# iden3/snarkjs

Hardware: NVIDIA H100
Metric: groth16_proofs_per_sec (higher is better)
Workload: dtype u32x8 (256-bit modular integers, 32-bit limbs)

## Files before the change

### snarkjs_b200/csrc/ec.cuh

```cuda
#pragma once
#include "fp.cuh"

namespace sb {

template <class P> struct Fp2 {
    typedef Fp<P> B;
    static constexpr bool HAS_MUL2 = false;
    B a, b;
    SB_HD static Fp2 one() { Fp2 r; r.a = B::one(); r.b = B::zero(); return r; }
    SB_HD static Fp2 inv(const Fp2& x) {
        B t = B::inv_binary(B::add(B::sqr(x.a), B::sqr(x.b)));
        Fp2 r; r.a = B::mul(x.a, t); r.b = B::neg(B::mul(x.b, t)); return r;
    }
    SB_HD static Fp2 zero() { Fp2 r; r.a = B::zero(); r.b = B::zero(); return r; }
    SB_HD bool is_zero() const { return a.is_zero() & b.is_zero(); }
    SB_HD bool operator==(const Fp2& o) const { return (a == o.a) & (b == o.b); }
    SB_HD static Fp2 add(const Fp2& x, const Fp2& y) { Fp2 r; r.a = B::add(x.a, y.a); r.b = B::add(x.b, y.b); return r; }
    SB_HD static Fp2 sub(const Fp2& x, const Fp2& y) { Fp2 r; r.a = B::sub(x.a, y.a); r.b = B::sub(x.b, y.b); return r; }
    SB_HD static Fp2 dbl(const Fp2& x) { Fp2 r; r.a = B::dbl(x.a); r.b = B::dbl(x.b); return r; }
    SB_HD static Fp2 neg(const Fp2& x) { Fp2 r; r.a = B::neg(x.a); r.b = B::neg(x.b); return r; }
    SB_HD static Fp2 cneg(const Fp2& x, bool f) { Fp2 r; r.a = B::cneg(x.a, f); r.b = B::cneg(x.b, f); return r; }
    SB_HD_NOINLINE static Fp2 mul(const Fp2& x, const Fp2& y) { return mul_i(x, y); }
    SB_HD_NOINLINE static Fp2 sqr(const Fp2& x) { return sqr_i(x); }
    SB_HD static Fp2 mul_i(const Fp2& x, const Fp2& y) {
#if defined(__CUDA_ARCH__) && defined(SB_FP2_LAZY)
        return mul_lazy(x, y);
#endif
        if constexpr (B::HAS_MUL2) {
            Fp2 r; r.a = B::mul2(x.a, y.a, x.b, B::neg(y.b)); r.b = B::mul2(x.a, y.b, x.b, y.a); return r;
        } else {
            B A = B::mul(x.a, y.a), Bb = B::mul(x.b, y.b);
            B C = B::mul(B::add(x.a, x.b), B::add(y.a, y.b));
            Fp2 r; r.a = B::sub(A, Bb); r.b = B::sub(B::sub(C, A), Bb); return r;
        }
    }
    SB_HD static Fp2 mul_lazy(const Fp2& x, const Fp2& y) {
        constexpr int N = B::N;
        uint32_t v0[2 * N], v1[2 * N], v2[2 * N], sa[N], sb[N];
        B::mul_wide(x.a.v, y.a.v, v0);
        B::mul_wide(x.b.v, y.b.v, v1);
        B::add_noreduce(x.a, x.b, sa); B::add_noreduce(y.a, y.b, sb);
        B::mul_wide(sa, sb, v2);
        B::wide_sub(v2, v0); B::wide_sub(v2, v1);
        uint32_t bw = B::wide_sub(v0, v1);
        B::wide_add_p_high(v0, bw);
        Fp2 r; r.a = B::redc_wide(v0); r.b = B::redc_wide(v2); return r;
    }
    SB_HD static Fp2 sqr_i(const Fp2& x) {
        B AB = B::mul(x.a, x.b);
        Fp2 r; r.a = B::mul(B::add(x.a, x.b), B::sub(x.a, x.b)); r.b = B::dbl(AB); return r;
    }
};

template <class F> struct Affine {
    F x, y;
    SB_HD bool is_inf() const { return x.is_zero() & y.is_zero(); }
};

template <class F> struct XYZZ {
    F x, y, zz, zzz;
    SB_HD static XYZZ inf() { XYZZ r; r.x = F::zero(); r.y = F::zero(); r.zz = F::zero(); r.zzz = F::zero(); return r; }
    SB_HD bool is_inf() const { return zz.is_zero(); }

    SB_HD_NOINLINE static XYZZ dbl_affine(const F& px, const F& py, const F& one) {
        XYZZ r;
        if (py.is_zero()) return inf();
        F U = F::dbl(py), V = F::sqr(U), W = F::mul(U, V), S = F::mul(px, V);
        F M = F::sqr(px); M = F::add(F::dbl(M), M);
        r.x = F::sub(F::sqr(M), F::dbl(S));
        r.y = F::sub(F::mul(M, F::sub(S, r.x)), F::mul(W, py));
        r.zz = V; r.zzz = W;
        (void)one;
        return r;
    }
    SB_HD_NOINLINE static XYZZ dbl(const XYZZ& p) {
        if (p.is_inf() || p.y.is_zero()) return inf();
        XYZZ r;
        F U = F::dbl(p.y), V = F::sqr(U), W = F::mul(U, V), S = F::mul(p.x, V);
        F M = F::sqr(p.x); M = F::add(F::dbl(M), M);
        r.x = F::sub(F::sqr(M), F::dbl(S));
        r.y = F::sub(F::mul(M, F::sub(S, r.x)), F::mul(W, p.y));
        r.zz = F::mul(V, p.zz); r.zzz = F::mul(W, p.zzz);
        return r;
    }
    SB_HD void add_affine(const F& qx, const F& qy, const F& one) {
        if (is_inf()) { x = qx; y = qy; zz = one; zzz = one; return; }
        F U2 = F::mul_i(qx, zz), S2 = F::mul_i(qy, zzz);
        F Pp = F::sub(U2, x), R = F::sub(S2, y);
        if (Pp.is_zero()) {
            if (R.is_zero()) *this = dbl_affine(qx, qy, one);
            else *this = inf();
            return;
        }
        F PP = F::sqr_i(Pp), PPP = F::mul_i(Pp, PP), Q = F::mul_i(x, PP);
        F X3 = F::sub(F::sub(F::sqr_i(R), PPP), F::dbl(Q));
        F Y3;
        if constexpr (F::HAS_MUL2) Y3 = F::mul2_i(R, F::sub(Q, X3), F::neg(y), PPP);
        else Y3 = F::sub(F::mul_i(R, F::sub(Q, X3)), F::mul_i(y, PPP));
        x = X3; y = Y3; zz = F::mul_i(zz, PP); zzz = F::mul_i(zzz, PPP);
    }
    SB_HD void add(const XYZZ& q) {
        if (q.is_inf()) return;
        if (is_inf()) { *this = q; return; }
        F U1 = F::mul(x, q.zz), U2 = F::mul(q.x, zz);
        F S1 = F::mul(y, q.zzz), S2 = F::mul(q.y, zzz);
        F Pp = F::sub(U2, U1), R = F::sub(S2, S1);
        if (Pp.is_zero()) {
            if (R.is_zero()) *this = dbl(*this);
            else *this = inf();
            return;
        }
        F PP = F::sqr(Pp), PPP = F::mul(Pp, PP), Q = F::mul(U1, PP);
        F X3 = F::sub(F::sub(F::sqr(R), PPP), F::dbl(Q));
        F Y3 = F::sub(F::mul(R, F::sub(Q, X3)), F::mul(S1, PPP));
        x = X3; y = Y3;
        zz = F::mul(F::mul(zz, q.zz), PP); zzz = F::mul(F::mul(zzz, q.zzz), PPP);
    }
};

}
```

### snarkjs_b200/csrc/msm.cuh

```cuda
#pragma once
#include <cuda_runtime.h>
#include "ec.cuh"
#include "msm_geom.h"

namespace sb {

static constexpr int MSM_SEG = 32;
static constexpr int MSM_ACC_THREADS = 128;
static constexpr int MSM_RED_CHUNK = 16;
static constexpr uint32_t MSM_INVALID_KEY = 0xffffffffu;
static constexpr int MSM_COUNTS_SEG = 8;


__host__ inline MsmGeom msm_choose(uint64_t n, uint32_t scalar_bytes, int fr_bits, bool precomp) {
    int eff = (int)(8 * scalar_bytes) < fr_bits ? (int)(8 * scalar_bytes) : fr_bits;
    int best_c = 3; double best = 1e300;
    for (int c = 3; c <= 22; c++) {
        int weff = (eff + 1 + c - 1) / c, top = eff + 1 - (weff - 1) * c;
        if (weff > 1 && top < c - 5) continue;
        double buckets = (precomp ? 1.0 : (double)weff) * (double)(1u << (c - 1));
        double cost = (double)weff * (double)n * 10.0 + buckets * 60.0;
        if (cost < best) { best = cost; best_c = c; }
    }
    MsmGeom g; g.c = best_c; g.W = (int)((8 * scalar_bytes + 1 + best_c - 1) / best_c); g.B = 1u << (best_c - 1);
    return g;
}
__host__ inline MsmGeom msm_geometry_precomp(uint64_t n_set, uint32_t scalar_bytes, int fr_bits = 254) {
    int l2 = 0; while ((1ull << (l2 + 1)) <= n_set) l2++;
    int cmax = l2; if (cmax > 22) cmax = 22; if (cmax < 8) cmax = 8;
    int c = 8;
    for (int cc = cmax; cc >= 8; cc--) {
        int weff = (fr_bits + 1 + cc - 1) / cc, top = fr_bits + 1 - (weff - 1) * cc;
        if (weff > 1 && top < cc - 5) continue;
        c = cc; break;
    }
    MsmGeom g; g.c = c; g.W = (int)((8 * scalar_bytes + 1 + c - 1) / c); g.B = 1u << (c - 1);
    g.precomp = 1; g.stride = n_set; g.first = 0;
    return g;
}
__host__ inline MsmGeom msm_geometry(uint64_t n, uint32_t scalar_bytes, int fr_bits = 254) {
    return msm_choose(n, scalar_bytes, fr_bits, false);
}

template <class F> __device__ __forceinline__ void load_affine(const Affine<F>* __restrict__ bases, uint32_t idx, F& x, F& y) {
    constexpr int NV = sizeof(F) / 16;
    const uint4* p = reinterpret_cast<const uint4*>(bases + idx);
    uint4* dx = reinterpret_cast<uint4*>(&x);
    uint4* dy = reinterpret_cast<uint4*>(&y);
#pragma unroll
    for (int k = 0; k < NV; k++) dx[k] = __ldg(p + k);
#pragma unroll
    for (int k = 0; k < NV; k++) dy[k] = __ldg(p + NV + k);
}
template <class T> __device__ __forceinline__ void store_vec(T* dst, const T& v) {
    constexpr int NV = sizeof(T) / 16;
    const uint4* s = reinterpret_cast<const uint4*>(&v);
    uint4* d = reinterpret_cast<uint4*>(dst);
#pragma unroll
    for (int k = 0; k < NV; k++) d[k] = s[k];
}
template <class T> __device__ __forceinline__ T load_vec(const T* src) {
    constexpr int NV = sizeof(T) / 16;
    T v; const uint4* s = reinterpret_cast<const uint4*>(src);
    uint4* d = reinterpret_cast<uint4*>(&v);
#pragma unroll
    for (int k = 0; k < NV; k++) d[k] = s[k];
    return v;
}

template <class P> __device__ __forceinline__ Fp<P> PairInvF(const Fp<P>& a) { return Fp<P>::inv_binary(a); }
template <class P> __device__ __forceinline__ Fp2<P> PairInvF(const Fp2<P>& a) { return Fp2<P>::inv(a); }

template <class F, int MINB>
__global__ void __launch_bounds__(MSM_ACC_THREADS, MINB)
k_accumulate(const Affine<F>* __restrict__ bases, const uint32_t* __restrict__ keys, const uint32_t* __restrict__ vals,
             const uint64_t* __restrict__ counts, XYZZ<F>* __restrict__ buckets,
             XYZZ<F>* __restrict__ heads, uint32_t* __restrict__ head_keys) {
    const uint64_t M = counts[0];
    const uint32_t seg = (uint32_t)counts[MSM_COUNTS_SEG];
    uint64_t t = blockIdx.x * (uint64_t)blockDim.x + threadIdx.x;
    uint64_t lo = t * seg;
    if (lo >= M) return;
    uint64_t hi = lo + seg < M ? lo + seg : M;
    const F one = F::one();
    XYZZ<F> acc = XYZZ<F>::inf();
    uint32_t cur = keys[lo];
    bool first = true;
    for (uint64_t e = lo; e < hi; e++) {
        uint32_t k = keys[e], v = vals ? vals[e] : (uint32_t)e;
        if (k != cur) {
            if (first) { store_vec(heads + t, acc); head_keys[t] = cur; first = false; }
            else store_vec(buckets + cur, acc);
            acc = XYZZ<F>::inf(); cur = k;
        }
        F px, py;
        load_affine<F>(bases, v & 0x7fffffffu, px, py);
        if (!(px.is_zero() & py.is_zero())) {
            py = F::cneg(py, (v >> 31) != 0);
            acc.add_affine(px, py, one);
        }
    }
    if (first) { store_vec(heads + t, acc); head_keys[t] = cur; }
    else store_vec(buckets + cur, acc);
}

static constexpr int MSM_SHORT_RUN = 8;
template <class F>
__global__ void __launch_bounds__(MSM_ACC_THREADS)
k_fold_short(const XYZZ<F>* __restrict__ heads, const uint32_t* __restrict__ keys_in, uint32_t* __restrict__ keys_out,
             const uint64_t* __restrict__ counts, XYZZ<F>* __restrict__ buckets) {
    const uint64_t M = counts[1];
    uint64_t t = blockIdx.x * (uint64_t)blockDim.x + threadIdx.x;
    if (t >= M) return;
    const uint32_t k = keys_in[t];
    uint64_t start = t; int back = 0;
    while (start > 0 && back < MSM_SHORT_RUN && keys_in[start - 1] == k) { start--; back++; }
    bool is_short = back < MSM_SHORT_RUN;
    uint64_t len = 0;
    if (is_short) {
        len = 1;
        while (start + len < M && len <= (uint64_t)MSM_SHORT_RUN && keys_in[start + len] == k) len++;
        is_short = len <= (uint64_t)MSM_SHORT_RUN;
    }
    keys_out[t] = is_short ? MSM_INVALID_KEY : k;
    if (!is_short || start != t) return;
    XYZZ<F> acc = load_vec(buckets + k);
    for (uint64_t e = 0; e < len; e++) { XYZZ<F> p = load_vec(heads + t + e); acc.add(p); }
    store_vec(buckets + k, acc);
}

template <class F>
__global__ void __launch_bounds__(MSM_ACC_THREADS)
k_fold(const XYZZ<F>* __restrict__ in, const uint32_t* __restrict__ in_keys, const uint64_t* __restrict__ counts, int level,
       XYZZ<F>* __restrict__ buckets, XYZZ<F>* __restrict__ heads, uint32_t* __restrict__ head_keys) {
    const uint64_t M = counts[level];
    const bool last = M <= MSM_SEG;
    uint64_t t = blockIdx.x * (uint64_t)blockDim.x + threadIdx.x;
    uint64_t lo = t * MSM_SEG;
    if (lo >= M) return;
    uint64_t hi = lo + MSM_SEG < M ? lo + MSM_SEG : M;
    XYZZ<F> acc = XYZZ<F>::inf();
    uint32_t cur = in_keys[lo];
    bool first = !last;
    auto flush = [&]() {
        if (first) { store_vec(heads + t, acc); head_keys[t] = cur; first = false; }
        else if (cur != MSM_INVALID_KEY) { XYZZ<F> b = load_vec(buckets + cur); b.add(acc); store_vec(buckets + cur, b); }
    };
    for (uint64_t e = lo; e < hi; e++) {
        uint32_t k = in_keys[e];
        if (k != cur) { flush(); acc = XYZZ<F>::inf(); cur = k; }
        if (k != MSM_INVALID_KEY) { XYZZ<F> p = load_vec(in + e); acc.add(p); }
    }
    flush();
}

template <class F>
__global__ void __launch_bounds__(128)
k_reduce(const XYZZ<F>* __restrict__ buckets, MsmGeom g, XYZZ<F>* __restrict__ partials, uint32_t ctas_per_window) {
    extern __shared__ uint4 smem_raw[];
    XYZZ<F>* sm = reinterpret_cast<XYZZ<F>*>(smem_raw);
    const uint32_t w = blockIdx.x / ctas_per_window, cta = blockIdx.x % ctas_per_window;
    const uint32_t L = g.B < (uint32_t)MSM_RED_CHUNK ? g.B : MSM_RED_CHUNK;
    const uint32_t chunks = g.B / L;
    const uint32_t j = cta * blockDim.x + threadIdx.x;
    XYZZ<F> part = XYZZ<F>::inf();
    if (j < chunks) {
        const XYZZ<F>* bk = buckets + (uint64_t)w * g.B + (uint64_t)j * L;
        XYZZ<F> run = XYZZ<F>::inf(), sum = XYZZ<F>::inf();
        for (int b = (int)L - 1; b >= 0; b--) {
            XYZZ<F> p = load_vec(bk + b);
            run.add(p);
            sum.add(run);
        }
        uint32_t k = j * L;
        if (k) {
            int top = 31 - __clz(k);
            part = run;
            for (int bit = top - 1; bit >= 0; bit--) {
                part = XYZZ<F>::dbl(part);
                if ((k >> bit) & 1) part.add(run);
            }
        }
        part.add(sum);
    }
    store_vec(sm + threadIdx.x, part);
    __syncthreads();
    for (uint32_t s = blockDim.x >> 1; s > 0; s >>= 1) {
        if (threadIdx.x < s) {
            XYZZ<F> a = load_vec(sm + threadIdx.x), b = load_vec(sm + threadIdx.x + s);
            a.add(b);
            store_vec(sm + threadIdx.x, a);
        }
        __syncthreads();
    }
    if (threadIdx.x == 0) store_vec(partials + (uint64_t)w * ctas_per_window + cta, load_vec(sm));
}

template <class F>
__global__ void __launch_bounds__(32)
k_window_sum(const XYZZ<F>* __restrict__ partials, uint32_t per_window, XYZZ<F>* __restrict__ out) {
    extern __shared__ uint4 smem_raw[];
    XYZZ<F>* sm = reinterpret_cast<XYZZ<F>*>(smem_raw);
    XYZZ<F> acc = XYZZ<F>::inf();
    for (uint32_t i = threadIdx.x; i < per_window; i += 32) { XYZZ<F> p = load_vec(partials + (uint64_t)blockIdx.x * per_window + i); acc.add(p); }
    store_vec(sm + threadIdx.x, acc);
    __syncwarp();
    for (uint32_t s = 16; s > 0; s >>= 1) {
        if (threadIdx.x < s) { XYZZ<F> a = load_vec(sm + threadIdx.x), b = load_vec(sm + threadIdx.x + s); a.add(b); store_vec(sm + threadIdx.x, a); }
        __syncwarp();
    }
    if (threadIdx.x == 0) store_vec(out + blockIdx.x, load_vec(sm));
}

template <class F> __device__ __noinline__ void padd(XYZZ<F>& a, const XYZZ<F>& b) { a.add(b); }

struct AxisJob { const void* in; void* out; uint64_t total; uint32_t S; uint32_t log_inner; };

template <class F>
__global__ void __launch_bounds__(128)
k_axis_sum(AxisJob j0, AxisJob j1) {
    const AxisJob j = blockIdx.y ? j1 : j0;
    const uint64_t gid = blockIdx.x * (uint64_t)blockDim.x + threadIdx.x;
    if (gid >= j.total) return;
    const uint64_t o = gid >> j.log_inner, i = gid & ((1ull << j.log_inner) - 1);
    const XYZZ<F>* p = (const XYZZ<F>*)j.in + ((o * j.S) << j.log_inner) + i;
    XYZZ<F> acc = load_vec(p);
#pragma unroll 1
    for (uint32_t s = 1; s < j.S; s++) { XYZZ<F> v = load_vec(p + ((uint64_t)s << j.log_inner)); acc.add(v); }
    store_vec((XYZZ<F>*)j.out + gid, acc);
}

template <class F> __device__ __forceinline__ XYZZ<F> shfl_down_pt(const XYZZ<F>& v, int d) {
    constexpr int NW32 = sizeof(XYZZ<F>) / 4;
    union U { XYZZ<F> p; uint32_t w[NW32]; __device__ U() {} };
    U a, r; a.p = v;
#pragma unroll
    for (int k = 0; k < NW32; k++) r.w[k] = __shfl_down_sync(0xffffffffu, a.w[k], d);
    return r.p;
}
template <class F> __device__ __forceinline__ void warp_weighted_sum(XYZZ<F> v, XYZZ<F>& T, XYZZ<F>& W) {
    const int lane = threadIdx.x & 31;
#pragma unroll 1
    for (int d = 1; d < 32; d <<= 1) { XYZZ<F> o = shfl_down_pt<F>(v, d); if (lane + d < 32) v.add(o); }
    T = v;
    XYZZ<F> x = lane ? v : XYZZ<F>::inf();
#pragma unroll 1
    for (int d = 16; d >= 1; d >>= 1) { XYZZ<F> o = shfl_down_pt<F>(x, d); if (lane < d) x.add(o); }
    W = x;
}
template <class F> __device__ __forceinline__ XYZZ<F> warp_sum(XYZZ<F> x) {
    const int lane = threadIdx.x & 31;
#pragma unroll 1
    for (int d = 16; d >= 1; d >>= 1) { XYZZ<F> o = shfl_down_pt<F>(x, d); if (lane < d) x.add(o); }
    return x;
}

template <class F>
__global__ void __launch_bounds__(128)
k_ws_chunks(const XYZZ<F>* __restrict__ vecR, uint32_t lenR, const XYZZ<F>* __restrict__ vecC, uint32_t lenC, uint32_t NW, XYZZ<F>* __restrict__ tw) {
    const uint32_t nR = (lenR + 31) / 32, nC = (lenC + 31) / 32, per = nR + nC;
    const uint32_t wid = blockIdx.x * (blockDim.x >> 5) + (threadIdx.x >> 5), lane = threadIdx.x & 31;
    if (wid >= NW * per) return;
    const uint32_t w = wid / per, jj = wid % per;
    const bool isR = jj < nR;
    const uint32_t j = isR ? jj : jj - nR, len = isR ? lenR : lenC, idx = j * 32 + lane;
    const XYZZ<F>* vec = (isR ? vecR : vecC) + (uint64_t)w * len;
    XYZZ<F> v = XYZZ<F>::inf();
    if (idx < len) v = load_vec(vec + idx);
    XYZZ<F> T, W;
    warp_weighted_sum<F>(v, T, W);
    if (lane == 0) { store_vec(tw + 2 * (uint64_t)wid, T); store_vec(tw + 2 * (uint64_t)wid + 1, W); }
}

template <class F>
__global__ void __launch_bounds__(128)
k_ws_final(const XYZZ<F>* __restrict__ tw, uint32_t nR, uint32_t nC, XYZZ<F>* __restrict__ out) {
    const uint32_t warp = threadIdx.x >> 5, lane = threadIdx.x & 31, per = nR + nC;
    const XYZZ<F>* base = tw + 2 * (uint64_t)blockIdx.x * per;
    const bool r_side = warp < 2;
    const uint32_t cnt = r_side ? nR : nC, off = r_side ? 0 : nR;
    XYZZ<F> v = XYZZ<F>::inf();
    if (lane < cnt) v = load_vec(base + 2 * (uint64_t)(off + lane) + (warp & 1));
    XYZZ<F>* o = out + 5 * (uint64_t)blockIdx.x;
    if ((warp & 1) == 0) {
        XYZZ<F> tot, res;
        warp_weighted_sum<F>(v, tot, res);
        if (lane == 0) { store_vec(o + (r_side ? 0 : 2), res); if (!r_side) store_vec(o + 4, tot); }
    } else {
        XYZZ<F> res = warp_sum<F>(v);
        if (lane == 0) store_vec(o + (r_side ? 1 : 3), res);
    }
}

template <class F>
__global__ void __launch_bounds__(128)
k_axis_tree(AxisJob j0, AxisJob j1) {
    const AxisJob j = blockIdx.y ? j1 : j0;
    const uint64_t wid = blockIdx.x * (uint64_t)(blockDim.x >> 5) + (threadIdx.x >> 5);
    const uint32_t lane = threadIdx.x & 31;
    if (wid >= j.total) return;
    const uint64_t o = wid >> j.log_inner, i = wid & ((1ull << j.log_inner) - 1);
    const XYZZ<F>* p = (const XYZZ<F>*)j.in + ((o * j.S) << j.log_inner) + i;
    XYZZ<F> acc = XYZZ<F>::inf();
#pragma unroll 1
    for (uint32_t s = lane; s < j.S; s += 32) { XYZZ<F> v = load_vec(p + ((uint64_t)s << j.log_inner)); acc.add(v); }
    acc = warp_sum<F>(acc);
    if (lane == 0) store_vec((XYZZ<F>*)j.out + wid, acc);
}

static constexpr int WS_COL_BITS = 10;
struct WsPlan {
    bool ok = false;
    int m = 0, er = 0, ec = 0;
    int levels = 0; int br[8] = {0}, bc[8] = {0};
    uint32_t lenR = 0, lenC = 0, nR = 0, nC = 0;
    size_t rowA = 0, rowB = 0, colA = 0, colB = 0, tw = 0;
    size_t elems() const { return rowA + rowB + colA + colB + tw + 8; }
};
__host__ inline WsPlan ws_plan(const MsmGeom& g) {
    WsPlan p; const int cbits = g.c - 1; const size_t NW = g.windows();
    if (cbits > 2 * WS_COL_BITS || cbits < 0) return p;
    p.ok = true;
    if (cbits > WS_COL_BITS) { p.m = WS_COL_BITS; p.er = p.m; p.ec = cbits - p.m; p.lenR = 1u << p.ec; p.lenC = 1u << p.m; }
    else { p.lenR = 0; p.lenC = g.B; }
    int rr = p.er, rc = p.ec;
    for (int l = 0; l < 2 && (rr > 0 || rc > 0); l++) {
        p.levels++;
        p.br[l] = l == 0 ? (rr < 3 ? rr : 3) : rr; p.bc[l] = l == 0 ? (rc < 3 ? rc : 3) : rc; rr -= p.br[l]; rc -= p.bc[l];
        const size_t orow = p.br[l] ? (NW * g.B) >> (p.er - rr) : 0, ocol = p.bc[l] ? (NW * g.B) >> (p.ec - rc) : 0;
        if (l & 1) { p.rowB = orow; p.colB = ocol; } else { p.rowA = orow; p.colA = ocol; }
    }
    p.nR = (p.lenR + 31) / 32; p.nC = (p.lenC + 31) / 32;
    p.tw = 2 * NW * (p.nR + p.nC);
    return p;
}
__host__ inline size_t msm_reduce_scratch_elems(const MsmGeom& g) {
    const uint32_t NW = g.windows();
    const uint32_t L = g.B < (uint32_t)MSM_RED_CHUNK ? g.B : MSM_RED_CHUNK;
    const uint32_t ctas_per_window = (g.B / L + 127) / 128;
    const size_t legacy = (size_t)2 * NW * ctas_per_window;
    const WsPlan p = ws_plan(g);
    return (p.ok && p.elems() > legacy) ? p.elems() : legacy;
}

template <class F>
__global__ void __launch_bounds__(128) k_precompute(const Affine<F>* __restrict__ bases, uint64_t n, int c, int W, Affine<F>* __restrict__ table) {
    uint64_t i = blockIdx.x * (uint64_t)blockDim.x + threadIdx.x;
    if (i >= n) return;
    Affine<F> a = load_vec(bases + i);
    store_vec(table + i, a);
    if (a.is_inf()) {
        for (int w = 1; w < W; w++) store_vec(table + (uint64_t)w * n + i, a);
        return;
    }
    XYZZ<F> p; p.x = a.x; p.y = a.y; p.zz = F::one(); p.zzz = F::one();
    for (int w = 1; w < W; w++) {
        for (int j = 0; j < c; j++) p = XYZZ<F>::dbl(p);
        Affine<F> o;
        if (p.is_inf()) { o.x = F::zero(); o.y = F::zero(); }
        else { F t = PairInvF(F::mul(p.zz, p.zzz)); o.x = F::mul(p.x, F::mul(t, p.zzz)); o.y = F::mul(p.y, F::mul(t, p.zz)); p.x = o.x; p.y = o.y; p.zz = F::one(); p.zzz = F::one(); }
        store_vec(table + (uint64_t)w * n + i, o);
    }
}

__host__ __device__ inline uint64_t splitmix64(uint64_t x) {
    x += 0x9E3779B97F4A7C15ull; x = (x ^ (x >> 30)) * 0xBF58476D1CE4E5B9ull; x = (x ^ (x >> 27)) * 0x94D049BB133111EBull; return x ^ (x >> 31);
}
static constexpr uint64_t GEN_CHUNK = 4096;
template <class F>
__global__ void __launch_bounds__(128) k_gen_points(Affine<F> g, uint64_t seed, uint64_t n, Affine<F>* __restrict__ out) {
    uint64_t i = blockIdx.x * (uint64_t)blockDim.x + threadIdx.x;
    if (i >= n) return;
    const uint64_t c = i / GEN_CHUNK, j = i % GEN_CHUNK;
    const uint64_t k0 = (seed ^ 0x9E3779B97F4A7C15ull) + c * 0xD1B54A32D192ED03ull, kd = seed * 2654435761ull + 12345ull;
    uint64_t lo = j * kd, hi = __umul64hi(j, kd);
    lo += k0; hi += lo < k0 ? 1 : 0;
    const F one = F::one();
    XYZZ<F> r = XYZZ<F>::inf();
    for (int bit = 79; bit >= 0; bit--) {
        r = XYZZ<F>::dbl(r);
        const uint64_t wd = bit >= 64 ? hi : lo;
        if ((wd >> (bit & 63)) & 1) r.add_affine(g.x, g.y, one);
    }
    Affine<F> a;
    if (r.is_inf()) { a.x = F::zero(); a.y = F::zero(); }
    else { F t = PairInvF(F::mul(r.zz, r.zzz)); a.x = F::mul(r.x, F::mul(t, r.zzz)); a.y = F::mul(r.y, F::mul(t, r.zz)); }
    store_vec(out + i, a);
}

struct MsmScratch {
    void* p = nullptr; size_t cap = 0;
    void* get(size_t bytes) {
        if (bytes > cap) { if (p) cudaFree(p); p = nullptr; cap = 0; if (cudaMalloc(&p, bytes) != cudaSuccess) return nullptr; cap = bytes; }
        return p;
    }
    void release() { if (p) cudaFree(p); p = nullptr; cap = 0; }
};

extern int g_msm_force_reduce;

struct MsmLaunchStats {
    int launches = 0;
    cudaEvent_t* ev = nullptr; int nev = 0; int used = 0; int tag[128] = {0}; int cur_tag = 0;
};
enum { PROF_ACC_G1 = 1, PROF_ACC_G2 = 2, PROF_SORT = 3, PROF_FOLD = 4, PROF_REDUCE = 5, PROF_QAP = 6, PROF_NTT = 7, PROF_JOIN = 8 };
struct ProfScope {
    MsmLaunchStats* s; cudaStream_t st; int idx = -1;
    ProfScope(MsmLaunchStats* s_, int tag, cudaStream_t st_) : s(s_), st(st_) {
        if (s && s->ev && s->used + 2 <= s->nev && s->used / 2 < 128) { idx = s->used; s->used += 2; s->tag[idx / 2] = tag; cudaEventRecord(s->ev[idx], st); }
    }
    void end() { if (idx >= 0) { cudaEventRecord(s->ev[idx + 1], st); idx = -1; } }
    void end(cudaStream_t other) { st = other; end(); }
};

struct MsmSorted {
    const uint32_t* keys = nullptr; const uint32_t* vals = nullptr; const uint64_t* counts = nullptr;
    uint64_t n = 0, total = 0; MsmGeom g{};
    uint32_t seg_lo = MSM_SEG;
};

int msm_sort_entries(const uint8_t* d_scalars, uint32_t sbytes, uint64_t n, MsmGeom g, MsmScratch& scratch,
                     cudaStream_t stream, MsmSorted* out, MsmLaunchStats* stats);

template <class F>
int msm_buckets(const Affine<F>* d_bases, const MsmSorted& s, MsmScratch& scratch, cudaStream_t stream,
                XYZZ<F>* d_wsum, MsmLaunchStats* stats, cudaStream_t tail_stream = nullptr, cudaEvent_t ev_acc = nullptr) {
    const MsmGeom g = s.g;
    const uint32_t NW = g.windows();
    const uint64_t nbuckets = (uint64_t)NW * g.B;
    const uint64_t heads0 = (s.total + s.seg_lo - 1) / s.seg_lo;
    const uint64_t heads1 = (heads0 + MSM_SEG - 1) / MSM_SEG;
    const uint32_t L = g.B < (uint32_t)MSM_RED_CHUNK ? g.B : MSM_RED_CHUNK;
    const uint32_t chunks = g.B / L;
    const uint32_t red_threads = 128;
    const uint32_t ctas_per_window = (chunks + red_threads - 1) / red_threads;
    auto al = [](size_t x) { return (x + 255) & ~(size_t)255; };
    size_t o_buckets = 0;
    size_t o_headsA = o_buckets + al(nbuckets * sizeof(XYZZ<F>)), o_hkA = o_headsA + al(heads0 * sizeof(XYZZ<F>));
    size_t o_headsB = o_hkA + al(heads0 * 4), o_hkB = o_headsB + al(heads1 * sizeof(XYZZ<F>));
    size_t o_hkM = o_hkB + al(heads1 * 4);
    size_t o_part = o_hkM + al(heads0 * 4);
    size_t bytes = o_part + al(msm_reduce_scratch_elems(g) * sizeof(XYZZ<F>));
    uint8_t* base = (uint8_t*)scratch.get(bytes);
    if (!base) return (int)cudaErrorMemoryAllocation;
    XYZZ<F>* buckets = (XYZZ<F>*)(base + o_buckets);
    XYZZ<F>* headsA = (XYZZ<F>*)(base + o_headsA); uint32_t* hkA = (uint32_t*)(base + o_hkA);
    XYZZ<F>* headsB = (XYZZ<F>*)(base + o_headsB); uint32_t* hkB = (uint32_t*)(base + o_hkB);
    XYZZ<F>* partials = (XYZZ<F>*)(base + o_part);
    uint32_t* hkM = (uint32_t*)(base + o_hkM);
    int launches = 0;
    cudaMemsetAsync(buckets, 0, nbuckets * sizeof(XYZZ<F>), stream);
    if (heads0) {
        ProfScope prof(stats, stats ? stats->cur_tag : 0, stream);
        {
            const unsigned grid = (unsigned)((heads0 + MSM_ACC_THREADS - 1) / MSM_ACC_THREADS);
            constexpr int MINB = sizeof(F) > 32 ? 2 : 4;
            k_accumulate<F, MINB><<<grid, MSM_ACC_THREADS, 0, stream>>>(d_bases, s.keys, s.vals, s.counts, buckets, headsA, hkA);
            launches++;
        }
        prof.end();
        if (tail_stream && tail_stream != stream && ev_acc) {
            cudaEventRecord(ev_acc, stream); cudaStreamWaitEvent(tail_stream, ev_acc, 0); stream = tail_stream;
        }
        ProfScope pfold(stats, PROF_FOLD, stream);
        k_fold_short<F><<<(unsigned)((heads0 + MSM_ACC_THREADS - 1) / MSM_ACC_THREADS), MSM_ACC_THREADS, 0, stream>>>(
            headsA, hkA, hkM, s.counts, buckets); launches++;
        uint64_t m = heads0; int level = 1;
        XYZZ<F>* hin = headsA; uint32_t* kin = hkM; XYZZ<F>* hout = headsB; uint32_t* kout = hkB;
        while (true) {
            uint64_t threads = (m + MSM_SEG - 1) / MSM_SEG;
            k_fold<F><<<(unsigned)((threads + MSM_ACC_THREADS - 1) / MSM_ACC_THREADS), MSM_ACC_THREADS, 0, stream>>>(
                hin, kin, s.counts, level, buckets, hout, kout); launches++;
            if (m <= (uint64_t)MSM_SEG) break;
            m = threads; level++;
            XYZZ<F>* th = hin; hin = hout; hout = th; uint32_t* tk = kin; kin = kout; kout = tk;
            if (level >= 8) return (int)cudaErrorUnknown;
        }
        pfold.end();
    }
    if (!heads0 && tail_stream && tail_stream != stream && ev_acc) { cudaEventRecord(ev_acc, stream); cudaStreamWaitEvent(tail_stream, ev_acc, 0); stream = tail_stream; }
    ProfScope pred(stats, PROF_REDUCE, stream);
    const WsPlan wp = ws_plan(g);
    if (wp.ok && !g_msm_force_reduce) {
        XYZZ<F>* rowb[2] = {partials, partials + wp.rowA};
        XYZZ<F>* colb[2] = {partials + wp.rowA + wp.rowB, partials + wp.rowA + wp.rowB + wp.colA};
        XYZZ<F>* tw = partials + wp.rowA + wp.rowB + wp.colA + wp.colB;
        const XYZZ<F>* rin = buckets; const XYZZ<F>* cin = buckets;
        int rr = wp.er, rc = wp.ec;
        for (int l = 0; l < wp.levels; l++) {
            AxisJob jr{nullptr, nullptr, 0, 1, 0}, jc{nullptr, nullptr, 0, 1, 0};
            if (wp.br[l]) { rr -= wp.br[l]; jr = AxisJob{rin, rowb[l & 1], (uint64_t)nbuckets >> (wp.er - rr), 1u << wp.br[l], (uint32_t)rr}; rin = rowb[l & 1]; }
            if (wp.bc[l]) { rc -= wp.bc[l]; jc = AxisJob{cin, colb[l & 1], (uint64_t)nbuckets >> (wp.ec - rc), 1u << wp.bc[l], (uint32_t)wp.m}; cin = colb[l & 1]; }
            const uint64_t mx = jr.total > jc.total ? jr.total : jc.total;
            if (l == 0) k_axis_sum<F><<<dim3((unsigned)((mx + 127) / 128), 2), 128, 0, stream>>>(jr, jc);
            else k_axis_tree<F><<<dim3((unsigned)((mx + 3) / 4), 2), 128, 0, stream>>>(jr, jc);
            launches++;
        }
        const uint32_t per = wp.nR + wp.nC;
        k_ws_chunks<F><<<(NW * per + 3) / 4, 128, 0, stream>>>(wp.lenR ? rin : nullptr, wp.lenR, cin, wp.lenC, NW, tw); launches++;
        k_ws_final<F><<<NW, 128, 0, stream>>>(tw, wp.nR, wp.nC, d_wsum); launches++;
    } else {
        k_reduce<F><<<NW * ctas_per_window, red_threads, red_threads * sizeof(XYZZ<F>), stream>>>(buckets, g, partials, ctas_per_window); launches++;
        k_window_sum<F><<<NW, 32, 32 * sizeof(XYZZ<F>), stream>>>(partials, ctas_per_window, d_wsum); launches++;
    }
    pred.end();
    if (stats) stats->launches += launches;
    return (int)cudaGetLastError();
}

}
```

Measured before the change: 40.63.

## Inline XYZZ add, add minBlocks launch bounds, and simplify tail reductions

Rewrites the generic XYZZ point add to use the inlined field mul/sqr variants and the fused mul2 path. It precomputes ZZ/ZZZ and feeds the doubling case the normalized point. It adds minimum-blocks launch bounds to the fold, axis and weighted-sum kernels, switches load/store helpers to union-based vector copies to avoid address-taken locals, and restructures the warp weighted-sum into suffix-sum plus shared warp_sum calls. The goal is to cut call overhead and local-memory spills in the MSM tail kernels. The cost is higher register pressure from inlining, which the launch bounds may turn into spills, plus two extra field muls per add when the points are equal.

```diff
diff --git a/snarkjs_b200/csrc/ec.cuh b/snarkjs_b200/csrc/ec.cuh
--- a/snarkjs_b200/csrc/ec.cuh
+++ b/snarkjs_b200/csrc/ec.cuh
@@ -102,19 +102,20 @@
     SB_HD void add(const XYZZ& q) {
         if (q.is_inf()) return;
         if (is_inf()) { *this = q; return; }
-        F U1 = F::mul(x, q.zz), U2 = F::mul(q.x, zz);
-        F S1 = F::mul(y, q.zzz), S2 = F::mul(q.y, zzz);
-        F Pp = F::sub(U2, U1), R = F::sub(S2, S1);
+        F U1 = F::mul_i(x, q.zz), S1 = F::mul_i(y, q.zzz);
+        F Pp = F::sub(F::mul_i(q.x, zz), U1), R = F::sub(F::mul_i(q.y, zzz), S1);
+        F ZZ = F::mul_i(zz, q.zz), ZZZ = F::mul_i(zzz, q.zzz);
         if (Pp.is_zero()) {
-            if (R.is_zero()) *this = dbl(*this);
+            if (R.is_zero()) { XYZZ t; t.x = U1; t.y = S1; t.zz = ZZ; t.zzz = ZZZ; *this = dbl(t); }
             else *this = inf();
             return;
         }
-        F PP = F::sqr(Pp), PPP = F::mul(Pp, PP), Q = F::mul(U1, PP);
-        F X3 = F::sub(F::sub(F::sqr(R), PPP), F::dbl(Q));
-        F Y3 = F::sub(F::mul(R, F::sub(Q, X3)), F::mul(S1, PPP));
-        x = X3; y = Y3;
-        zz = F::mul(F::mul(zz, q.zz), PP); zzz = F::mul(F::mul(zzz, q.zzz), PPP);
+        F PP = F::sqr_i(Pp), PPP = F::mul_i(Pp, PP), Q = F::mul_i(U1, PP);
+        F X3 = F::sub(F::sub(F::sqr_i(R), PPP), F::dbl(Q));
+        F Y3;
+        if constexpr (F::HAS_MUL2) Y3 = F::mul2_i(R, F::sub(Q, X3), F::neg(S1), PPP);
+        else Y3 = F::sub(F::mul_i(R, F::sub(Q, X3)), F::mul_i(S1, PPP));
+        x = X3; y = Y3; zz = F::mul_i(ZZ, PP); zzz = F::mul_i(ZZZ, PPP);
     }
 };
 
diff --git a/snarkjs_b200/csrc/msm.cuh b/snarkjs_b200/csrc/msm.cuh
--- a/snarkjs_b200/csrc/msm.cuh
+++ b/snarkjs_b200/csrc/msm.cuh
@@ -10,6 +10,7 @@
 static constexpr int MSM_RED_CHUNK = 16;
 static constexpr uint32_t MSM_INVALID_KEY = 0xffffffffu;
 static constexpr int MSM_COUNTS_SEG = 8;
+template <class F> constexpr int MSM_TAIL_MINB = sizeof(F) == 32 ? 3 : 2;
 
 
 __host__ inline MsmGeom msm_choose(uint64_t n, uint32_t scalar_bytes, int fr_bits, bool precomp) {
@@ -42,30 +43,30 @@
     return msm_choose(n, scalar_bytes, fr_bits, false);
 }
 
+template <class T> union Vec16 { T v; uint4 u[sizeof(T) / 16]; __device__ Vec16() {} };
 template <class F> __device__ __forceinline__ void load_affine(const Affine<F>* __restrict__ bases, uint32_t idx, F& x, F& y) {
     constexpr int NV = sizeof(F) / 16;
     const uint4* p = reinterpret_cast<const uint4*>(bases + idx);
-    uint4* dx = reinterpret_cast<uint4*>(&x);
-    uint4* dy = reinterpret_cast<uint4*>(&y);
+    Vec16<F> dx, dy;
 #pragma unroll
-    for (int k = 0; k < NV; k++) dx[k] = __ldg(p + k);
+    for (int k = 0; k < NV; k++) dx.u[k] = __ldg(p + k);
 #pragma unroll
-    for (int k = 0; k < NV; k++) dy[k] = __ldg(p + NV + k);
+    for (int k = 0; k < NV; k++) dy.u[k] = __ldg(p + NV + k);
+    x = dx.v; y = dy.v;
 }
 template <class T> __device__ __forceinline__ void store_vec(T* dst, const T& v) {
     constexpr int NV = sizeof(T) / 16;
-    const uint4* s = reinterpret_cast<const uint4*>(&v);
+    Vec16<T> s; s.v = v;
     uint4* d = reinterpret_cast<uint4*>(dst);
 #pragma unroll
-    for (int k = 0; k < NV; k++) d[k] = s[k];
+    for (int k = 0; k < NV; k++) d[k] = s.u[k];
 }
 template <class T> __device__ __forceinline__ T load_vec(const T* src) {
     constexpr int NV = sizeof(T) / 16;
-    T v; const uint4* s = reinterpret_cast<const uint4*>(src);
-    uint4* d = reinterpret_cast<uint4*>(&v);
+    Vec16<T> d; const uint4* s = reinterpret_cast<const uint4*>(src);
 #pragma unroll
-    for (int k = 0; k < NV; k++) d[k] = s[k];
-    return v;
+    for (int k = 0; k < NV; k++) d.u[k] = s[k];
+    return d.v;
 }
 
 template <class P> __device__ __forceinline__ Fp<P> PairInvF(const Fp<P>& a) { return Fp<P>::inv_binary(a); }
@@ -106,7 +107,7 @@
 
 static constexpr int MSM_SHORT_RUN = 8;
 template <class F>
-__global__ void __launch_bounds__(MSM_ACC_THREADS)
+__global__ void __launch_bounds__(MSM_ACC_THREADS, MSM_TAIL_MINB<F>)
 k_fold_short(const XYZZ<F>* __restrict__ heads, const uint32_t* __restrict__ keys_in, uint32_t* __restrict__ keys_out,
              const uint64_t* __restrict__ counts, XYZZ<F>* __restrict__ buckets) {
     const uint64_t M = counts[1];
@@ -130,7 +131,7 @@
 }
 
 template <class F>
-__global__ void __launch_bounds__(MSM_ACC_THREADS)
+__global__ void __launch_bounds__(MSM_ACC_THREADS, MSM_TAIL_MINB<F>)
 k_fold(const XYZZ<F>* __restrict__ in, const uint32_t* __restrict__ in_keys, const uint64_t* __restrict__ counts, int level,
        XYZZ<F>* __restrict__ buckets, XYZZ<F>* __restrict__ heads, uint32_t* __restrict__ head_keys) {
     const uint64_t M = counts[level];
@@ -212,12 +213,10 @@
     if (threadIdx.x == 0) store_vec(out + blockIdx.x, load_vec(sm));
 }
 
-template <class F> __device__ __noinline__ void padd(XYZZ<F>& a, const XYZZ<F>& b) { a.add(b); }
-
 struct AxisJob { const void* in; void* out; uint64_t total; uint32_t S; uint32_t log_inner; };
 
 template <class F>
-__global__ void __launch_bounds__(128)
+__global__ void __launch_bounds__(MSM_ACC_THREADS, MSM_TAIL_MINB<F>)
 k_axis_sum(AxisJob j0, AxisJob j1) {
     const AxisJob j = blockIdx.y ? j1 : j0;
     const uint64_t gid = blockIdx.x * (uint64_t)blockDim.x + threadIdx.x;
@@ -238,15 +237,11 @@
     for (int k = 0; k < NW32; k++) r.w[k] = __shfl_down_sync(0xffffffffu, a.w[k], d);
     return r.p;
 }
-template <class F> __device__ __forceinline__ void warp_weighted_sum(XYZZ<F> v, XYZZ<F>& T, XYZZ<F>& W) {
+template <class F> __device__ __forceinline__ XYZZ<F> warp_suffix_sum(XYZZ<F> v) {
     const int lane = threadIdx.x & 31;
 #pragma unroll 1
     for (int d = 1; d < 32; d <<= 1) { XYZZ<F> o = shfl_down_pt<F>(v, d); if (lane + d < 32) v.add(o); }
-    T = v;
-    XYZZ<F> x = lane ? v : XYZZ<F>::inf();
-#pragma unroll 1
-    for (int d = 16; d >= 1; d >>= 1) { XYZZ<F> o = shfl_down_pt<F>(x, d); if (lane < d) x.add(o); }
-    W = x;
+    return v;
 }
 template <class F> __device__ __forceinline__ XYZZ<F> warp_sum(XYZZ<F> x) {
     const int lane = threadIdx.x & 31;
@@ -256,7 +251,7 @@
 }
 
 template <class F>
-__global__ void __launch_bounds__(128)
+__global__ void __launch_bounds__(MSM_ACC_THREADS, MSM_TAIL_MINB<F>)
 k_ws_chunks(const XYZZ<F>* __restrict__ vecR, uint32_t lenR, const XYZZ<F>* __restrict__ vecC, uint32_t lenC, uint32_t NW, XYZZ<F>* __restrict__ tw) {
     const uint32_t nR = (lenR + 31) / 32, nC = (lenC + 31) / 32, per = nR + nC;
     const uint32_t wid = blockIdx.x * (blockDim.x >> 5) + (threadIdx.x >> 5), lane = threadIdx.x & 31;
@@ -267,13 +262,14 @@
     const XYZZ<F>* vec = (isR ? vecR : vecC) + (uint64_t)w * len;
     XYZZ<F> v = XYZZ<F>::inf();
     if (idx < len) v = load_vec(vec + idx);
-    XYZZ<F> T, W;
-    warp_weighted_sum<F>(v, T, W);
-    if (lane == 0) { store_vec(tw + 2 * (uint64_t)wid, T); store_vec(tw + 2 * (uint64_t)wid + 1, W); }
-}
-
-template <class F>
-__global__ void __launch_bounds__(128)
+    v = warp_suffix_sum<F>(v);
+    if (lane == 0) store_vec(tw + 2 * (uint64_t)wid, v);
+    v = warp_sum<F>(lane ? v : XYZZ<F>::inf());
+    if (lane == 0) store_vec(tw + 2 * (uint64_t)wid + 1, v);
+}
+
+template <class F>
+__global__ void __launch_bounds__(MSM_ACC_THREADS, MSM_TAIL_MINB<F>)
 k_ws_final(const XYZZ<F>* __restrict__ tw, uint32_t nR, uint32_t nC, XYZZ<F>* __restrict__ out) {
     const uint32_t warp = threadIdx.x >> 5, lane = threadIdx.x & 31, per = nR + nC;
     const XYZZ<F>* base = tw + 2 * (uint64_t)blockIdx.x * per;
@@ -283,17 +279,16 @@
     if (lane < cnt) v = load_vec(base + 2 * (uint64_t)(off + lane) + (warp & 1));
     XYZZ<F>* o = out + 5 * (uint64_t)blockIdx.x;
     if ((warp & 1) == 0) {
-        XYZZ<F> tot, res;
-        warp_weighted_sum<F>(v, tot, res);
-        if (lane == 0) { store_vec(o + (r_side ? 0 : 2), res); if (!r_side) store_vec(o + 4, tot); }
-    } else {
-        XYZZ<F> res = warp_sum<F>(v);
-        if (lane == 0) store_vec(o + (r_side ? 1 : 3), res);
-    }
-}
-
-template <class F>
-__global__ void __launch_bounds__(128)
+        v = warp_suffix_sum<F>(v);
+        if (lane == 0 && !r_side) store_vec(o + 4, v);
+        if (lane == 0) v = XYZZ<F>::inf();
+    }
+    v = warp_sum<F>(v);
+    if (lane == 0) store_vec(o + (r_side ? 0 : 2) + (warp & 1), v);
+}
+
+template <class F>
+__global__ void __launch_bounds__(MSM_ACC_THREADS, MSM_TAIL_MINB<F>)
 k_axis_tree(AxisJob j0, AxisJob j1) {
     const AxisJob j = blockIdx.y ? j1 : j0;
     const uint64_t wid = blockIdx.x * (uint64_t)(blockDim.x >> 5) + (threadIdx.x >> 5);
```

After: 41.33 (median of 6 runs). 1.02x the previous value.
